# A-Andrews/Muzero-Hanoi

Measured on AMD Instinct MI355X. Metric: MCTS sims/sec (node) 4-disk Hanoi, 50 sims/move, 65k root batch; 1/2/4/8 GPU, higher is better.
Workload: dtype fp32

## Files before the change

muzero-hanoi_amd/csrc/mzh_wave.hip:

```cpp
#include "mzh_device.h"
#include "mzh_internal.h"
#include "mzh_mcts.h"

#define MZW_WAVES 4
#define MZW_DC 16

struct MzwNX {
  uint16_t N;
  int16_t X;
};
struct __align__(128) MzwBlock {
  MzwNX nx[6];
  float R[6];
  float P[6];
  double W[6];
  uint32_t pad[2];
};
static_assert(sizeof(MzwBlock) == 128, "block layout");

template <int ROOTS>
struct MzwWave {
  double rW[6][ROOTS];
  double rP[6][ROOTS];
  float rR[6][ROOTS];
  int rN[6][ROOTS];
  int rX[6][ROOTS];
  double pcW[MZW_DC][ROOTS];
  float pcR[MZW_DC][ROOTS];
  int pcN[MZW_DC][ROOTS];
  uint16_t path[MZW_DC][ROOTS];
};

static __host__ __device__ inline size_t mzw_hdr_bytes(int S) {
  size_t b = sizeof(float) * MZH_A * MZH_F + sizeof(double) * 2 * (size_t)(S + 3);
  return (b + 15) & ~(size_t)15;
}

__device__ __forceinline__ void mzw_wave_sync() {
  __builtin_amdgcn_fence(__ATOMIC_RELEASE, "wavefront");
  __builtin_amdgcn_wave_barrier();
  __builtin_amdgcn_fence(__ATOMIC_ACQUIRE, "wavefront");
}

__device__ __forceinline__ float mzw_max4g(float v) {
  float a, b;
  mzh_pair16(v, a, b);
  v = __builtin_fmaxf(a, b);
  mzh_pair32(v, a, b);
  return __builtin_fmaxf(a, b);
}
__device__ __forceinline__ float mzw_min4g(float v) {
  float a, b;
  mzh_pair16(v, a, b);
  v = __builtin_fminf(a, b);
  mzh_pair32(v, a, b);
  return __builtin_fminf(a, b);
}
__device__ __forceinline__ float mzw_add16(float v) {
  float a, b;
  mzh_pair16(v, a, b);
  return a + b;
}
__device__ __forceinline__ float mzw_add32(float v) {
  float a, b;
  mzh_pair32(v, a, b);
  return a + b;
}

__device__ __forceinline__ floatx4 mzw_ld4(__amdgpu_buffer_rsrc_t r, int voff, int soff) {
  return __builtin_bit_cast(floatx4, __builtin_amdgcn_raw_buffer_load_b128(r, voff, soff, 0));
}

template <int NT, int KB1, int NO, bool OH, bool B32 = false, int WS = 0>
__device__ __forceinline__ void mzw_chain(const MzhWMlp& L, __amdgpu_buffer_rsrc_t rw, const floatx4 (&x)[NT][4],
                                          const float* const (&oh)[NT], floatx4 (&out)[NO][NT], floatx4* b2, int lane,
                                          float* p32 = nullptr, floatx4* wst = nullptr, int next_soff = 0) {
  constexpr int FR = KB1 + NO;
  static_assert(WS == 0 || WS >= FR, "chained buffer too small");
  const int g = lane >> 4;
  const int vs = 16 * lane, vb = 16 * g;
#pragma unroll
  for (int ot = 0; ot < NO; ++ot)
#pragma unroll
    for (int n = 0; n < NT; ++n) out[ot][n] = floatx4{0.f, 0.f, 0.f, 0.f};
  floatx4 wloc[WS > 0 ? 1 : FR];
  floatx4* w = WS > 0 ? wst : wloc;
  if constexpr (WS == 0) {
#pragma unroll
    for (int f = 0; f < FR; ++f) w[f] = mzw_ld4(rw, vs, L.soff + f * 1024);
  }
#pragma unroll
  for (int ot = 0; ot < NO; ++ot) b2[ot] = mzw_ld4(rw, vb, L.b2off + 64 * ot);
  float a32[NT];
#pragma unroll
  for (int n = 0; n < NT; ++n) a32[n] = 0.0f;
#pragma unroll 2
  for (int ht = 0; ht < 16; ++ht) {
    const int sn = (WS > 0 && ht == 15) ? next_soff : L.soff + (ht + 1) * FR * 1024;
    const floatx4 b = mzw_ld4(rw, vb, L.b1off + 64 * ht);
    floatx4 w32 = {0.f, 0.f, 0.f, 0.f};
    if (B32) w32 = mzw_ld4(rw, vb, L.w32off + 64 * ht);
    floatx4 o[NT];
#pragma unroll
    for (int n = 0; n < NT; ++n)
      o[n] = OH ? *reinterpret_cast<const floatx4*>(oh[n] + 16 * ht) : floatx4{0.f, 0.f, 0.f, 0.f};
    floatx4 acc[NT];
#pragma unroll
    for (int n = 0; n < NT; ++n) acc[n] = floatx4{0.f, 0.f, 0.f, 0.f};
#pragma unroll
    for (int kb = 0; kb < KB1; ++kb) {
#pragma unroll
      for (int t = 0; t < 4; ++t)
#pragma unroll
        for (int n = 0; n < NT; ++n)
          acc[n] = __builtin_amdgcn_mfma_f32_16x16x4f32(w[kb][t], x[n][kb][t], acc[n], 0, 0, 0);
      w[kb] = mzw_ld4(rw, vs, sn + kb * 1024);
      __builtin_amdgcn_sched_barrier(0);
    }
    floatx4 hid[NT];
#pragma unroll
    for (int n = 0; n < NT; ++n) {
#pragma unroll
      for (int i = 0; i < 4; ++i) {
        float v = acc[n][i];
        if (OH) v = v + o[n][i];
        v = v + b[i];
        hid[n][i] = v > 0.0f ? v : 0.0f;
      }
    }
#pragma unroll
    for (int t = 0; t < 4; ++t) {
#pragma unroll
      for (int ot = 0; ot < NO; ++ot)
#pragma unroll
        for (int n = 0; n < NT; ++n)
          out[ot][n] = __builtin_amdgcn_mfma_f32_16x16x4f32(w[KB1 + ot][t], hid[n][t], out[ot][n], 0, 0, 0);
      if (B32) {
#pragma unroll
        for (int n = 0; n < NT; ++n) a32[n] = __builtin_fmaf(hid[n][t], w32[t], a32[n]);
        if (NT > 1) asm("" : "+v"(a32[0]));
      }
    }
#pragma unroll
    for (int ot = 0; ot < NO; ++ot) w[KB1 + ot] = mzw_ld4(rw, vs, sn + (KB1 + ot) * 1024);
    __builtin_amdgcn_sched_barrier(0);
  }
  if constexpr (WS > FR) {
#pragma unroll
    for (int f = FR; f < WS; ++f) w[f] = mzw_ld4(rw, vs, next_soff + f * 1024);
  }
  if (B32) {
#pragma unroll
    for (int n = 0; n < NT; ++n) p32[n] = a32[n];
  }
}

template <int NT, int NO>
__device__ __forceinline__ void mzw_bias2(floatx4 (&out)[NO][NT], const floatx4* b2) {
#pragma unroll
  for (int ot = 0; ot < NO; ++ot) {
    const floatx4 b = b2[ot];
#pragma unroll
    for (int n = 0; n < NT; ++n)
#pragma unroll
      for (int i = 0; i < 4; ++i) out[ot][n][i] = out[ot][n][i] + b[i];
  }
}

template <int NT>
__device__ __forceinline__ void mzw_normalize(const floatx4 (&hp)[4][NT], int n, floatx4 (&hn)[NT][4]) {
  float mn = hp[0][n][0], mx = hp[0][n][0];
#pragma unroll
  for (int ot = 0; ot < 4; ++ot)
#pragma unroll
    for (int i = 0; i < 4; ++i) {
      const float v = hp[ot][n][i];
      mn = __builtin_fminf(v, mn);
      mx = __builtin_fmaxf(v, mx);
    }
  mn = mzw_min4g(mn);
  mx = mzw_max4g(mx);
  const float d = (mx - mn) + 9.999999939225290290778502821922302246094e-09f;
  const float y = 1.0f / d;
  const float lim = __builtin_fmaxf(d < __builtin_inff() ? d * 0x1p-99f : 0.0f, 0x1p-100f);
  unsigned amin = 0xFFFFFFFFu;
#pragma unroll
  for (int ot = 0; ot < 4; ++ot)
#pragma unroll
    for (int i = 0; i < 4; ++i) {
      const float a = hp[ot][n][i] - mn;
      amin = min(amin, __float_as_uint(a) - 1u);
      const float q = a * y;
      hn[n][ot][i] = __builtin_fmaf(__builtin_fmaf(-q, d, a), y, q);
    }
  const bool slow = amin < __float_as_uint(lim) - 1u;
  if (__builtin_expect(__ballot(slow) != 0, 0)) {
#pragma unroll
    for (int ot = 0; ot < 4; ++ot)
#pragma unroll
      for (int i = 0; i < 4; ++i) hn[n][ot][i] = (hp[ot][n][i] - mn) / d;
  }
}

template <int NT, int NO>
__device__ __forceinline__ float mzw_head(const floatx4 (&l)[NO][NT], int n, int lane, float p32 = 0.0f,
                                          float b32 = 0.0f) {
  const int g = lane >> 4;
  if constexpr (NO == 1) {
    return __shfl(l[0][n][0], lane & 15);
  } else {
  static_assert(NO == 2, "33-bin heads: two tiles + the bin-32 chains");
  const bool v8 = g == 0;
  float L[9];
#pragma unroll
  for (int s = 0; s < 8; ++s) L[s] = l[s >> 2][n][s & 3];
  L[8] = mzw_add32(mzw_add16(p32)) + b32;
  float m = L[0];
#pragma unroll
  for (int s = 1; s < 8; ++s) m = __builtin_fmaxf(L[s], m);
  if (v8) m = __builtin_fmaxf(L[8], m);
  m = mzw_max4g(m);
  float e[9];
#pragma unroll
  for (int s = 0; s < 8; ++s) e[s] = mzh_expf_np(L[s] - m);
  e[8] = mzh_expf_np(L[8] - m);
  e[8] = v8 ? e[8] : 0.0f;
  float s0 = e[0];
  s0 = s0 + e[2];
  s0 = s0 + e[4];
  s0 = s0 + e[6];
  if (v8) s0 = s0 + e[8];
  float s1 = e[1];
  s1 = s1 + e[3];
  s1 = s1 + e[5];
  s1 = s1 + e[7];
  float t = s0 + s1;
  t = mzw_add16(t);
  t = mzw_add32(t);
  const float y = 1.0f / t;
  float lmin = L[0];
#pragma unroll
  for (int s = 1; s < 8; ++s) lmin = __builtin_fminf(L[s], lmin);
  if (v8) lmin = __builtin_fminf(L[8], lmin);
  const bool slow = lmin - m < -65.0f;
  float pk[9];
#pragma unroll
  for (int s = 0; s < 9; ++s) {
    const float q = e[s] * y;
    pk[s] = __builtin_fmaf(__builtin_fmaf(-q, t, e[s]), y, q);
  }
  if (__builtin_expect(__ballot(slow) != 0, 0)) {
#pragma unroll
    for (int s = 0; s < 9; ++s) pk[s] = e[s] / t;
  }
  float pr[9];
#pragma unroll
  for (int s = 0; s < 9; ++s) pr[s] = pk[s] * (float)(2 * g + (s & 1) + 8 * (s >> 1) - 16);
  float x0 = pr[0];
  x0 = x0 + pr[2];
  x0 = x0 + pr[4];
  x0 = x0 + pr[6];
  if (v8) x0 = x0 + pr[8];
  float x1 = pr[1];
  x1 = x1 + pr[3];
  x1 = x1 + pr[5];
  x1 = x1 + pr[7];
  float xs = x0 + x1;
  xs = mzw_add16(xs);
  xs = mzw_add32(xs);
  return mzh_signed_parabolic(xs);
  }
}

__device__ __forceinline__ floatx4 mzw_policy(const floatx4 l, int lane) {
  const int g = lane >> 4;
  const bool ok01 = g < 2, ok23 = g == 0;
  float m = -__builtin_inff();
  if (ok01) {
    m = __builtin_fmaxf(l[0], m);
    m = __builtin_fmaxf(l[1], m);
  }
  if (ok23) {
    m = __builtin_fmaxf(l[2], m);
    m = __builtin_fmaxf(l[3], m);
  }
  m = mzw_max4g(m);
  const float x0 = mzh_expf_np(l[0] - m), x1 = mzh_expf_np(l[1] - m);
  const float x2 = mzh_expf_np(l[2] - m), x3 = mzh_expf_np(l[3] - m);
  const float e0 = ok01 ? x0 : 0.0f, e1 = ok01 ? x1 : 0.0f;
  const float e2 = ok23 ? x2 : 0.0f, e3 = ok23 ? x3 : 0.0f;
  float t = (e0 + e1) + (e2 + e3);
  t = mzw_add16(t);
  const float y = 1.0f / t;
  float lmin = __builtin_inff();
  if (ok01) lmin = __builtin_fminf(__builtin_fminf(l[0], l[1]), lmin);
  if (ok23) lmin = __builtin_fminf(__builtin_fminf(l[2], l[3]), lmin);
  const bool slow = lmin - m < -65.0f;
  auto mdiv = [&](float a) {
    const float q = a * y;
    return __builtin_fmaf(__builtin_fmaf(-q, t, a), y, q);
  };
  floatx4 p;
  p[0] = mdiv(e0);
  p[1] = mdiv(e1);
  p[2] = mdiv(e2);
  p[3] = mdiv(e3);
  if (__builtin_expect(__ballot(slow) != 0, 0)) {
    p[0] = e0 / t;
    p[1] = e1 / t;
    p[2] = e2 / t;
    p[3] = e3 / t;
  }
  return p;
}

__device__ __forceinline__ int mzw_pick_pair(const float (&u)[3], int half, int tie, int& firstTie, int& extra) {
  float m = u[0];
  m = __builtin_fmaxf(u[1], m);
  m = __builtin_fmaxf(u[2], m);
  float a, b;
  mzh_pair32(m, a, b);
  const float M = __builtin_fmaxf(a, b);
  int mask = 0;
#pragma unroll
  for (int j = 0; j < 3; ++j) mask |= (u[j] == M ? 1 : 0) << j;
  mask <<= 3 * half;
  const auto r = __builtin_amdgcn_permlane32_swap((unsigned)mask, (unsigned)mask, false, false);
  return mzh_tie_pick(r[0] | r[1], tie, firstTie, extra);
}

template <int NC>
struct MzwCols {
  int root[NC];
  bool valid[NC];
  int en[NC], an[NC];
  int prow[NC];
  float val[NC], rew[NC];
  floatx4 cpi[NC];
};

template <int NT, bool REPLAY, bool SUP33>
__global__ __launch_bounds__(MZW_WAVES * 64, 2) void mzh_wave_kernel(MzhWNet net, MzhSearchParams p) {
  constexpr int NOV = SUP33 ? 2 : 1;
  constexpr int ROOTS = 16 * NT;
  const float* const noh[NT] = {};
  extern __shared__ __align__(16) unsigned char smem_raw[];
  const int S = p.S;
  float* ohl = reinterpret_cast<float*>(smem_raw);
  double* table = reinterpret_cast<double*>(smem_raw + sizeof(float) * MZH_A * MZH_F);
  MzwWave<ROOTS>* wsa = reinterpret_cast<MzwWave<ROOTS>*>(smem_raw + mzw_hdr_bytes(S));
  const int tid = threadIdx.x, lane = tid & 63;
  const int wave = __builtin_amdgcn_readfirstlane(tid >> 6);
  const int g = lane >> 4, col = lane & 15;
  const __amdgpu_buffer_rsrc_t rw = mzh_rsrc(net.wbase);

  if (!REPLAY)
    for (int i = tid; i < MZH_A * MZH_F; i += MZW_WAVES * 64) ohl[i] = net.oh[i];
  double* inv = table + (S + 3);
  for (int i = tid; i < S + 3; i += MZW_WAVES * 64) {
    table[i] = i < S + 2 ? p.table[i] : 0.0;
    inv[i] = 1.0 / (double)i;
  }
  __syncthreads();
  const int wr0 = (blockIdx.x * MZW_WAVES + wave) * ROOTS;
  if (wr0 >= p.B) return;
  MzwWave<ROOTS>& ws = wsa[wave];
  const double disc = p.discount;
  const bool noised = p.noise != nullptr;
  const size_t E = (size_t)p.E;

  const int rho = lane & 31;
  const int half = lane >> 5;
  const int rroot = wr0 + rho;
  const bool rvalid = rho < ROOTS && rroot < p.B;
  const int tb0 = (rvalid ? rroot : 0) * p.E;
  auto TB = [&](int e) -> MzwBlock& { return reinterpret_cast<MzwBlock*>(p.tree)[(size_t)(unsigned)(tb0 + e)]; };
  MzhMinMax mm;
  if (rvalid && p.minmax_in)
    mm.set(p.minmax_in[2 * rroot], p.minmax_in[2 * rroot + 1]);
  else
    mm.set(-__builtin_inf(), __builtin_inf());
  int firstTie = 0, extra = 0, steps = 0, rootN = 0, depth = 0;
  int leaf = 0;
  int lsum = 0;
  double rootW = 0.0;
  const int tie = (rvalid && p.tie_idx) ? p.tie_idx[rroot] : 0;
  const bool memo = !REPLAY && p.memo_h != nullptr;
  int sigma = -1;
  unsigned pid = 0;
  unsigned cnt = 0;
  const bool grow = memo && p.memo_link != nullptr;
  const bool glog = grow && p.memo_log != nullptr && p.memo_ctr[0] < p.memo_cap;
  if (memo && rvalid) {
    const unsigned* orow = reinterpret_cast<const unsigned*>(p.obs) + (size_t)rroot * p.in_dim;
    int sg = 0, w3 = 1;
    bool ok = true;
    for (int i = 0; 3 * i + 2 < p.in_dim; ++i, w3 *= 3) {
      const unsigned a0 = orow[3 * i], a1 = orow[3 * i + 1], a2 = orow[3 * i + 2];
      const unsigned one = 0x3F800000u;
      const int n1 = (a0 == one) + (a1 == one) + (a2 == one), n0 = (a0 == 0u) + (a1 == 0u) + (a2 == 0u);
      ok = ok && n1 == 1 && n0 == 2;
      sg += w3 * (a1 == one ? 1 : a2 == one ? 2 : 0);
    }
    sigma = ok ? sg : -1;
  }

  int croot[NT];
  bool cvalid[NT];
#pragma unroll
  for (int n = 0; n < NT; ++n) {
    croot[n] = wr0 + 16 * n + col;
    cvalid[n] = croot[n] < p.B;
  }

  floatx4 rpi[NT];
  const bool rtab = memo && __ballot(rvalid && sigma < 0) == 0;
  if (!REPLAY && rtab) {
#pragma unroll
    for (int n = 0; n < NT; ++n) {
      const int sg = __shfl(sigma, 16 * n + col);
      rpi[n] = floatx4{0.f, 0.f, 0.f, 0.f};
      if (cvalid[n] && g < 2) {
        const float* rec = p.memo_rec + (size_t)sg * p.memo_K * 8 + 4 * g;
        if (g == 0) {
          rpi[n] = *reinterpret_cast<const floatx4*>(rec);
        } else {
          rpi[n][0] = rec[0];
          rpi[n][1] = rec[1];
        }
      }
    }
  } else if (!REPLAY) {
    floatx4 hreg[NT][4];
    floatx4 x[NT][4];
#pragma unroll
    for (int n = 0; n < NT; ++n)
#pragma unroll
      for (int kb = 0; kb < 4; ++kb)
#pragma unroll
        for (int t = 0; t < 4; ++t) {
          const int k = 16 * kb + 4 * t + g;
          x[n][kb][t] = (cvalid[n] && k < p.in_dim) ? p.obs[(size_t)croot[n] * p.in_dim + k] : 0.0f;
        }
    floatx4 hp[4][NT];
    floatx4 b2[4];
    switch (net.rep.kb1) {
      case 1: mzw_chain<NT, 1, 4, false>(net.rep, rw, x, noh, hp, b2, lane); break;
      case 2: mzw_chain<NT, 2, 4, false>(net.rep, rw, x, noh, hp, b2, lane); break;
      case 3: mzw_chain<NT, 3, 4, false>(net.rep, rw, x, noh, hp, b2, lane); break;
      default: mzw_chain<NT, 4, 4, false>(net.rep, rw, x, noh, hp, b2, lane); break;
    }
    mzw_bias2<NT, 4>(hp, b2);
#pragma unroll
    for (int n = 0; n < NT; ++n) {
      mzw_normalize<NT>(hp, n, hreg);
      if (cvalid[n]) {
        floatx4* dst = reinterpret_cast<floatx4*>(p.htree + ((size_t)croot[n] * E) * MZH_H) + g;
#pragma unroll
        for (int kb = 0; kb < 4; ++kb) dst[4 * kb] = hreg[n][kb];
      }
    }
    floatx4 pl[1][NT];
    mzw_chain<NT, 4, 1, false>(net.pol, rw, hreg, noh, pl, b2, lane);
    mzw_bias2<NT, 1>(pl, b2);
    floatx4 vl[NOV][NT];
    mzw_chain<NT, 4, NOV, false>(net.val, rw, hreg, noh, vl, b2, lane);
    (void)vl;
#pragma unroll
    for (int n = 0; n < NT; ++n) rpi[n] = mzw_policy(pl[0][n], lane);
  }
  if (g < 2) {
#pragma unroll
    for (int n = 0; n < NT; ++n)
#pragma unroll
      for (int i = 0; i < 4; ++i) {
        const int c = 4 * g + i;
        if (c < MZH_A && cvalid[n]) {
          const float pr = REPLAY ? p.rp_root_pi[(size_t)croot[n] * MZH_A + c] : rpi[n][i];
          ws.rP[c][16 * n + col] =
              mzh_root_prior(pr, noised, p.eps, noised ? p.noise[(size_t)croot[n] * MZH_A + c] : 0.0);
        }
      }
  }
  if (lane < ROOTS) {
#pragma unroll
    for (int c = 0; c < MZH_A; ++c) {
      ws.rW[c][rho] = 0.0;
      ws.rR[c][rho] = 0.0f;
      ws.rN[c][rho] = 0;
      ws.rX[c][rho] = -1;
    }
  }
  mzw_wave_sync();

  MzwCols<NT> cf;
#pragma unroll
  for (int n = 0; n < NT; ++n) {
    cf.root[n] = cvalid[n] ? croot[n] : 0;
    cf.valid[n] = cvalid[n];
    cf.prow[n] = -1;
  }
  MzwCols<1> cp;

  floatx4 wst[8];
  if (!REPLAY) {
#pragma unroll
    for (int f = 0; f < 8; ++f) wst[f] = mzw_ld4(rw, 16 * lane, net.dyn.soff + f * 1024);
  }
  MZH_STAMP_DECL
  auto phase_select = [&](int s, auto ex) {
    (void)s;
    constexpr bool exact = decltype(ex)::value;
    if (rvalid) {
      const bool has = mm.has();
      const double mmin = mm.mmin, den = mm.den, dinv = mm.dinv;
      float u[3];
      const double tr = table[rootN];
#pragma unroll
      for (int j = 0; j < 3; ++j) {
        const int c = 3 * half + j;
        u[j] = mzh_ucb(ws.rN[c][rho], ws.rW[c][rho], ws.rR[c][rho], ws.rP[c][rho], noised || p.np1, tr, disc, has,
                       mmin, den, dinv, inv, exact);
      }
      int pick = mzw_pick_pair(u, half, tie, firstTie, extra);
      int Np = ws.rN[pick][rho], X = ws.rX[pick][rho];
      ws.path[0][rho] = (uint16_t)pick;
      ws.pcW[0][rho] = ws.rW[pick][rho];
      ws.pcR[0][rho] = ws.rR[pick][rho];
      ws.pcN[0][rho] = Np;
      int e = 0, d = 1;
      pid = 0;
      constexpr bool kPF = NT == 1;
      int pf0 = 0, pf1 = 0, pf2 = 0;
      while (X >= 0 && d <= S) {
        e = X;
        pid = 6u * pid + (unsigned)pick + 1u;
        int nx;
        double Wp;
        float Rp;
        {
          const unsigned char* blk = reinterpret_cast<const unsigned char*>(&TB(e));
          const uint3 hnx = *reinterpret_cast<const uint3*>(blk + 12 * half);
          const uint3 hR = *reinterpret_cast<const uint3*>(blk + 24 + 12 * half);
          const uint3 hP = *reinterpret_cast<const uint3*>(blk + 48 + 12 * half);
          typedef unsigned int u32x4_a8 __attribute__((ext_vector_type(4), aligned(8)));
          const u32x4_a8 hW01 = *reinterpret_cast<const u32x4_a8*>(blk + 72 + 24 * half);
          const uint2 hW2 = *reinterpret_cast<const uint2*>(blk + 88 + 24 * half);
          const int hn[3] = {(int)hnx.x, (int)hnx.y, (int)hnx.z};
          const float hr[3] = {__uint_as_float(hR.x), __uint_as_float(hR.y), __uint_as_float(hR.z)};
          const float hp[3] = {__uint_as_float(hP.x), __uint_as_float(hP.y), __uint_as_float(hP.z)};
          const double hw[3] = {__hiloint2double((int)hW01.y, (int)hW01.x), __hiloint2double((int)hW01.w, (int)hW01.z),
                                __hiloint2double((int)hW2.y, (int)hW2.x)};
          if (kPF) {
            asm volatile("" ::"v"(pf0), "v"(pf1), "v"(pf2));
            const int x0 = hn[0] >> 16, x1 = hn[1] >> 16, x2 = hn[2] >> 16;
            pf0 = *reinterpret_cast<const int*>(&TB(x0 >= 0 ? x0 : e));
            pf1 = *reinterpret_cast<const int*>(&TB(x1 >= 0 ? x1 : e));
            pf2 = *reinterpret_cast<const int*>(&TB(x2 >= 0 ? x2 : e));
          }
          const double tn = table[Np];
  #pragma unroll
          for (int j = 0; j < 3; ++j) u[j] = mzh_ucb(hn[j] & 0xFFFF, hw[j], hr[j], (double)hp[j], p.np1, tn, disc, has, mmin, den, dinv, inv, exact);
          pick = mzw_pick_pair(u, half, tie, firstTie, extra);
          const int jl = pick - 3 * half;
          int cn = hn[0];
          float cr = hr[0];
          double cw = hw[0];
  #pragma unroll
          for (int q = 1; q < 3; ++q)
            if (jl == q) {
              cn = hn[q];
              cr = hr[q];
              cw = hw[q];
            }
          auto take = [&](unsigned v) {
            const auto r = __builtin_amdgcn_permlane32_swap(v, v, false, false);
            return pick >= 3 ? r[1] : r[0];
          };
          nx = (int)take((unsigned)cn);
          Rp = __uint_as_float(take(__float_as_uint(cr)));
          const long long wb = __double_as_longlong(cw);
          Wp = __hiloint2double((int)take((unsigned)(wb >> 32)), (int)take((unsigned)(wb & 0xFFFFFFFFll)));
        }
        Np = nx & 0xFFFF;
        X = nx >> 16;
        const uint16_t slot = (uint16_t)(e * 8 + pick);
        if (d < MZW_DC) {
          ws.path[d][rho] = slot;
          ws.pcW[d][rho] = Wp;
          ws.pcR[d][rho] = Rp;
          ws.pcN[d][rho] = Np;
        } else {
          p.pathx[(size_t)rroot * E + d] = slot;
        }
        ++d;
      }
      if (kPF) asm volatile("" ::"v"(pf0), "v"(pf1), "v"(pf2));
      depth = d;
      leaf = (leaf & ~0x3FFFF) | (e * 8 + pick);
      steps += d;
    }
    if (p.lockstep_levels) {
      int m = rvalid ? depth - 1 : 0;
#pragma unroll
      for (int off = 32; off > 0; off >>= 1) m = max(m, __shfl_xor(m, off));
      lsum += m;
    }
  };

  auto phase_mlp = [&](int s, auto& C) {
    if (REPLAY) return;
    constexpr int NC = sizeof(C.root) / sizeof(int);
    const float* const nohc[NC] = {};
    floatx4 rl[NOV][NC], pl[1][NC], vl[NOV][NC];
    floatx4 x[NC][4];
#pragma unroll
    for (int n = 0; n < NC; ++n) {
      const float* row = C.prow[n] >= 0 ? p.memo_h + (size_t)C.prow[n] * MZH_H
                                        : p.htree + ((size_t)C.root[n] * E + C.en[n]) * MZH_H;
      const floatx4* src = reinterpret_cast<const floatx4*>(row) + g;
#pragma unroll
      for (int kb = 0; kb < 4; ++kb) x[n][kb] = src[4 * kb];
    }
    floatx4 hreg[NC][4];
    floatx4 hp[4][NC];
    const float* ohp[NC];
#pragma unroll
    for (int n = 0; n < NC; ++n) ohp[n] = ohl + C.an[n] * MZH_F + 4 * g;
    MZH_STAMP(10);
    floatx4 b2[4];
    mzw_chain<NC, 4, 4, true, false, 8>(net.dyn, rw, x, ohp, hp, b2, lane, nullptr, wst, net.rwd.soff);
    mzw_bias2<NC, 4>(hp, b2);
    MZH_STAMP(5);
    floatx4 hx[NC][4];
#pragma unroll
    for (int n = 0; n < NC; ++n)
#pragma unroll
      for (int kb = 0; kb < 4; ++kb) hx[n][kb] = hp[kb][n];
    float r32[NC], v32[NC];
    mzw_chain<NC, 4, NOV, false, SUP33, 8>(net.rwd, rw, hx, nohc, rl, b2, lane, r32, wst, net.pol.soff);
    mzw_bias2<NC, NOV>(rl, b2);
    MZH_STAMP(6);
#pragma unroll
    for (int n = 0; n < NC; ++n) C.rew[n] = mzw_head<NC, NOV>(rl, n, lane, SUP33 ? r32[n] : 0.0f, net.rwd.b32);
    MZH_STAMP(11);
#pragma unroll
    for (int n = 0; n < NC; ++n) {
      mzw_normalize<NC>(hp, n, hreg);
      if (C.valid[n]) {
        floatx4* dst = reinterpret_cast<floatx4*>(p.htree + ((size_t)C.root[n] * E + s + 1) * MZH_H) + g;
#pragma unroll
        for (int kb = 0; kb < 4; ++kb) dst[4 * kb] = hreg[n][kb];
      }
    }
    MZH_STAMP(7);
    mzw_chain<NC, 4, 1, false, false, 8>(net.pol, rw, hreg, nohc, pl, b2, lane, nullptr, wst, net.val.soff);
    mzw_bias2<NC, 1>(pl, b2);
#pragma unroll
    for (int n = 0; n < NC; ++n) C.cpi[n] = mzw_policy(pl[0][n], lane);
    MZH_STAMP(8);
    mzw_chain<NC, 4, NOV, false, SUP33, 8>(net.val, rw, hreg, nohc, vl, b2, lane, v32, wst, net.dyn.soff);
    mzw_bias2<NC, NOV>(vl, b2);
    MZH_STAMP(9);
#pragma unroll
    for (int n = 0; n < NC; ++n) C.val[n] = mzw_head<NC, NOV>(vl, n, lane, SUP33 ? v32[n] : 0.0f, net.val.b32);
  };

  auto phase_blocks = [&](int s, auto& C, bool own, int hrow) {
    constexpr int NC = sizeof(C.root) / sizeof(int);
    unsigned trow[NC];
#pragma unroll
    for (int n = 0; n < NC; ++n) trow[n] = own ? (unsigned)(__shfl(hrow, 16 * n + col) + 1) : 0u;
#pragma unroll
    for (int n = 0; n < NC; ++n) {
      if (!C.valid[n]) continue;
      uint4* nb = reinterpret_cast<uint4*>(reinterpret_cast<MzwBlock*>(p.tree) + (size_t)C.root[n] * E + s + 1);
      const uint32_t nx = 0xFFFF0000u;
      uint4 c0, c1;
      if (g == 0) {
        c0 = make_uint4(nx, nx, nx, nx);
        c1 = make_uint4(__float_as_uint(C.cpi[n][0]), __float_as_uint(C.cpi[n][1]), __float_as_uint(C.cpi[n][2]),
                        __float_as_uint(C.cpi[n][3]));
      } else if (g == 1) {
        c0 = make_uint4(nx, nx, 0u, 0u);
        c1 = make_uint4(__float_as_uint(C.cpi[n][0]), __float_as_uint(C.cpi[n][1]), 0u, 0u);
      } else {
        c0 = make_uint4(0u, 0u, 0u, 0u);
        c1 = make_uint4(0u, 0u, g == 3 ? trow[n] : 0u, 0u);
      }
      const int k0 = g < 3 ? g : 6, k1 = g < 3 ? g + 3 : 7;
      nb[k0] = c0;
      nb[k1] = c1;
    }
  };

  auto phase_head = [&](int s, bool fromrec, float vcol, float rcol, int hrow) {
    if (rvalid) {
      const int enew = s + 1;
      const int leafE = (leaf & 0x3FFFF) >> 3, leafA = leaf & 7;
      float vv, rr;
      if (REPLAY || fromrec) {
        const uint4* rec = reinterpret_cast<const uint4*>(
            REPLAY ? p.rp_sim + ((size_t)s * p.B + rroot) * 8 : p.memo_rec + (size_t)hrow * 8);
        const uint4 r0 = rec[0], r1 = rec[1];
        rr = __uint_as_float(r1.z);
        vv = __uint_as_float(r1.w);
        uint4* nb = reinterpret_cast<uint4*>(&TB(enew));
        const uint32_t nx = 0xFFFF0000u;
        const uint4 z = make_uint4(0u, 0u, 0u, 0u);
        const uint4 c7 = REPLAY ? z : make_uint4(0u, 0u, (unsigned)(hrow + 1), 0u);
        const bool h1 = half != 0;
        const uint32_t nx0 = h1 ? 0u : nx;
        nb += 4 * half;
        nb[0] = make_uint4(h1 ? r1.x : nx, h1 ? r1.y : nx, nx0, nx0);
        nb[1] = make_uint4(nx0, nx0, 0u, 0u);
        nb[2] = z;
        nb[3] = make_uint4(h1 ? 0u : r0.x, h1 ? 0u : r0.y, h1 ? c7.z : r0.z, h1 ? 0u : r0.w);
      } else {
        vv = vcol;
        rr = rcol;
        if (!REPLAY && glog && sigma >= 0 && hrow < 0 && (leaf >> 18) < p.memo_logcap) {
          int ro = rroot;
          asm volatile("" : "+v"(ro));
          if (!half)
            p.memo_log[(unsigned)(ro * p.memo_logcap + (leaf >> 18))] =
                make_uint4((unsigned)enew, (unsigned)(leaf & 0x3FFFF), __float_as_uint(vv), __float_as_uint(rr));
          leaf += 1 << 18;
        }
      }
      const bool st = !half;
      if (st) {
        if (leafE == 0) {
          ws.rX[leafA][rho] = enew;
          ws.rR[leafA][rho] = rr;
        } else {
          TB(leafE).nx[leafA].X = (int16_t)enew;
          TB(leafE).R[leafA] = rr;
        }
      }
      MZH_STAMP(12);
      double v = (double)vv;
      double lmax = -__builtin_inf(), lmin = __builtin_inf();
      auto load_lds = [&](int j, int& slot, double& W, float& R, int& N) {
        slot = ws.path[j][rho];
        W = ws.pcW[j][rho];
        R = ws.pcR[j][rho];
        N = ws.pcN[j][rho];
      };
      auto load_hbm = [&](int j, int& slot, double& W, float& R, int& N) {
        slot = p.pathx[(size_t)rroot * E + j];
        const int e = slot >> 3, a = slot & 7;
        W = TB(e).W[a];
        R = TB(e).R[a];
        N = TB(e).nx[a].N;
      };
      int slot;
      double Wj;
      float Rj;
      int Nj;
      auto node = [&](int j, double& Wn, int& Nn) {
        const double rw = (j == depth - 1) ? (double)rr : (double)Rj;
        Wn = Wj + v;
        Nn = Nj + 1;
        const double q = rw + disc * mzh_div(Wn, (double)Nn, inv[Nn]);
        lmax = q > lmax ? q : lmax;
        lmin = q < lmin ? q : lmin;
        v = rw + disc * v;
      };
      if (depth - 1 < MZW_DC) load_lds(depth - 1, slot, Wj, Rj, Nj);
      else load_hbm(depth - 1, slot, Wj, Rj, Nj);
      int j = depth - 1;
      auto hbm_node = [&](int jn) {
        const int e = slot >> 3, a = slot & 7;
        double Wn;
        int Nn;
        node(jn, Wn, Nn);
        if (st) {
          TB(e).W[a] = Wn;
          TB(e).nx[a].N = (uint16_t)Nn;
        }
      };
      for (; j >= 1; --j) {
        int slot_n, Nj_n;
        double Wj_n;
        float Rj_n;
        if (j - 1 < MZW_DC) load_lds(j - 1, slot_n, Wj_n, Rj_n, Nj_n);
        else load_hbm(j - 1, slot_n, Wj_n, Rj_n, Nj_n);
        hbm_node(j);
        slot = slot_n;
        Wj = Wj_n;
        Rj = Rj_n;
        Nj = Nj_n;
      }
      {
        const int a = slot & 7;
        double Wn;
        int Nn;
        node(0, Wn, Nn);
        if (st) {
          ws.rW[a][rho] = Wn;
          ws.rN[a][rho] = Nn;
        }
      }
      rootW = rootW + v;
      rootN = rootN + 1;
      const double q = 0.0 + disc * mzh_div(rootW, (double)rootN, inv[rootN]);
      lmax = q > lmax ? q : lmax;
      lmin = q < lmin ? q : lmin;
      mm.update(lmax, lmin);
    }
  };

  for (int s = 0; s < S; ++s) {
    MZH_STAMP(4);
    if (__builtin_expect(mzh_need_exact(rvalid && mm.has(), mm.den), 0))
      phase_select(s, MzhBool<true>{});
    else
      phase_select(s, MzhBool<false>{});
    MZH_STAMP(0);
    __builtin_amdgcn_s_setprio(1);
    int mode = 2, nm = 0;
    unsigned mask = 0;
    bool hit = false;
    int prow_r = -1, hrow = -1;
    const int leafE = (leaf & 0x3FFFF) >> 3, leafA = leaf & 7;
    if (memo && sigma >= 0) {
      if (depth - 1 <= p.memo_D) prow_r = sigma * p.memo_K + (int)pid;
      else if (grow) prow_r = (int)TB(leafE).pad[0] - 1;
      if (depth <= p.memo_D) {
        hrow = sigma * p.memo_K + (int)(6u * pid + (unsigned)leafA + 1u);
      } else if (grow && prow_r >= 0) {
        const int l = p.memo_link[prow_r * 6 + leafA];
        hrow = l > 0 ? l : -1;
      }
    }
    if (memo) {
      hit = hrow >= 0;
      mask = __builtin_amdgcn_readfirstlane((unsigned)__ballot(rvalid && !hit));
      nm = __popc(mask);
      mode = nm == 0 ? 0 : (NT == 2 && nm <= 16) ? 1 : 2;
      cnt = __builtin_amdgcn_readfirstlane(cnt + (mode == 0 ? 1u : mode == 1 ? 0x10000u : 0u));
    }
    MZH_STAMP(3);
    float vcol = 0.0f, rcol = 0.0f;
    if (mode == 2) {
      if (!REPLAY) {
#pragma unroll
        for (int n = 0; n < NT; ++n) {
          const int lf = __shfl(leaf, 16 * n + col);
          cf.en[n] = (lf & 0x3FFFF) >> 3;
          cf.an[n] = lf & 7;
          if (memo) cf.prow[n] = __shfl(prow_r, 16 * n + col);
        }
        phase_mlp(s, cf);
        vcol = cf.val[0];
        rcol = cf.rew[0];
#pragma unroll
        for (int n = 1; n < NT; ++n)
          if ((rho >> 4) == n) {
            vcol = cf.val[n];
            rcol = cf.rew[n];
          }
      }
    } else if constexpr (NT == 2) {
     if (mode == 1) {
      const int rank = __popc(mask & ((1u << rho) - 1u));
      const bool missl = (mask >> rho) & 1u;
      const int dest = half ? lane : (missl ? rank : nm + rho - rank);
      const int rsel = __builtin_amdgcn_ds_permute(dest << 2, rho);
      const bool pv = col < nm;
      const int rs = __shfl(rsel, col);
      const int r = pv ? rs : (int)__builtin_ctz(mask);
      cp.root[0] = wr0 + r;
      cp.valid[0] = pv;
      const int lf = __shfl(leaf, r);
      cp.en[0] = (lf & 0x3FFFF) >> 3;
      cp.an[0] = lf & 7;
      cp.prow[0] = __shfl(prow_r, r);
      phase_mlp(s, cp);
      vcol = __shfl(cp.val[0], rank);
      rcol = __shfl(cp.rew[0], rank);
     }
    }
    __builtin_amdgcn_s_setprio(0);
    MZH_STAMP(1);
    if (!REPLAY) {
      if (mode == 2) phase_blocks(s, cf, true, hrow);
      else if (NT == 2 && mode == 1) phase_blocks(s, cp, false, -1);
    }
    phase_head(s, mode != 2 && hit, vcol, rcol, hrow);
    MZH_STAMP(2);
    __builtin_amdgcn_fence(__ATOMIC_ACQ_REL, "workgroup");
    __builtin_amdgcn_wave_barrier();
  }

  if (p.lockstep_levels && lane == 0) p.lockstep_levels[blockIdx.x * MZW_WAVES + wave] = lsum;
  if (memo && lane == 0) {
    const unsigned nskip = cnt & 0xFFFFu, npack = cnt >> 16;
    atomicAdd(p.memo_cnt + 0, (unsigned long long)nskip);
    atomicAdd(p.memo_cnt + 1, (unsigned long long)npack);
    atomicAdd(p.memo_cnt + 2, (unsigned long long)((unsigned)S - nskip - npack));
    if (p.memo_logn && blockIdx.x == 0 && wave == 0) p.memo_ctr[1] = p.memo_ctr[0];
  }
  if (!rvalid || half) return;
  if (!REPLAY && p.memo_logn) p.memo_logn[rroot] = leaf >> 18;
  int vis[MZH_A];
  for (int a = 0; a < MZH_A; ++a) vis[a] = ws.rN[a][rho];
  mzh_write_results(p, rroot, vis, rootW, rootN, mm.mmax, mm.mmin, extra, steps, depth, [&](int j) {
    return j < MZW_DC ? (int)ws.path[j][rho] : (int)p.pathx[(size_t)rroot * E + j];
  });
}

size_t mzh_wave_smem_bytes(int S, int nt) {
  return mzw_hdr_bytes(S) + (nt == 1 ? sizeof(MzwWave<16>) : sizeof(MzwWave<32>)) * MZW_WAVES;
}

template <int NT, bool REPLAY, bool SUP33>
static hipError_t launch_wave_t(const MzhWNet& net, const MzhSearchParams& p, hipStream_t stream) {
  const size_t smem = mzh_wave_smem_bytes(p.S, NT);
  hipError_t e = hipFuncSetAttribute(reinterpret_cast<const void*>(&mzh_wave_kernel<NT, REPLAY, SUP33>),
                                     hipFuncAttributeMaxDynamicSharedMemorySize, (int)smem);
  if (e != hipSuccess) return e;
  const int per_wg = MZW_WAVES * 16 * NT;
  const int grid = (p.B + per_wg - 1) / per_wg;
  hipLaunchKernelGGL((mzh_wave_kernel<NT, REPLAY, SUP33>), dim3(grid), dim3(MZW_WAVES * 64), smem, stream, net, p);
  return hipGetLastError();
}

template <int NT>
static hipError_t launch_wave_nt(const MzhSearchPlan& pl, const MzhWNet& net, const MzhSearchParams& p, hipStream_t stream) {
  if (pl.replay) return pl.sup33 ? launch_wave_t<NT, true, true>(net, p, stream) : launch_wave_t<NT, true, false>(net, p, stream);
  return pl.sup33 ? launch_wave_t<NT, false, true>(net, p, stream) : launch_wave_t<NT, false, false>(net, p, stream);
}

hipError_t mzh_launch_wave_search(const MzhSearchPlan& pl, const MzhWNet& net, const MzhSearchParams& p, hipStream_t stream) {
  return pl.nt == 1 ? launch_wave_nt<1>(pl, net, p, stream) : launch_wave_nt<2>(pl, net, p, stream);
}

__global__ __launch_bounds__(256) void mzh_memo_level_kernel(const float4* hprev, float4* xin, int32_t* act, long long n) {
  const long long i = (long long)blockIdx.x * 256 + threadIdx.x;
  if (i >= n * 16) return;
  const long long r = i >> 4;
  xin[i] = hprev[(r / 6) * 16 + (i & 15)];
  if ((i & 15) == 0) act[r] = (int32_t)(r % 6);
}
__global__ __launch_bounds__(256) void mzh_memo_scatter_kernel(const float* h, const float* pi, const float* reward,
                                                               const float* value, long long n, long long per_state,
                                                               long long K, long long first_id, float* memo_h,
                                                               float* memo_rec) {
  const long long i = (long long)blockIdx.x * 256 + threadIdx.x;
  if (i >= n * 64) return;
  const long long r = i >> 6;
  const int pos = (int)(i & 63);
  const long long row = (r / per_state) * K + first_id + (r % per_state);
  const int kb = pos >> 4, gg = (pos >> 2) & 3, t = pos & 3;
  memo_h[row * 64 + pos] = h[r * 64 + 16 * kb + 4 * t + gg];
  if (pos < 8) memo_rec[row * 8 + pos] = pos < 6 ? pi[r * 6 + pos] : pos == 6 ? reward[r] : value[r];
}
hipError_t mzh_launch_memo_level(const float* hprev, float* xin, int32_t* act, long long n, hipStream_t stream) {
  const long long blocks = (n * 16 + 255) / 256;
  hipLaunchKernelGGL(mzh_memo_level_kernel, dim3((unsigned)blocks), dim3(256), 0, stream,
                     reinterpret_cast<const float4*>(hprev), reinterpret_cast<float4*>(xin), act, n);
  return hipGetLastError();
}
hipError_t mzh_launch_memo_scatter(const float* h, const float* pi, const float* reward, const float* value, long long n,
                                   long long per_state, long long K, long long first_id, float* memo_h, float* memo_rec,
                                   hipStream_t stream) {
  const long long blocks = (n * 64 + 255) / 256;
  hipLaunchKernelGGL(mzh_memo_scatter_kernel, dim3((unsigned)blocks), dim3(256), 0, stream, h, pi, reward, value, n,
                     per_state, K, first_id, memo_h, memo_rec);
  return hipGetLastError();
}

__global__ __launch_bounds__(256) void mzh_memo_harvest_kernel(MzhHarvestParams h) {
  const int root = blockIdx.x * 256 + threadIdx.x;
  if (root >= h.B) return;
  int n = h.logn[root];
  if (n <= 0) return;
  n = min(n, h.logcap);
  MzwBlock* tb = reinterpret_cast<MzwBlock*>(h.tree) + (size_t)root * h.E;
  const uint4* log = h.log + (size_t)root * h.logcap;
  for (int i = 0; i < n; ++i) {
    const uint4 en = log[i];
    const int e = (int)en.x, pe = (int)(en.y >> 3), a = (int)(en.y & 7u);
    if (e < 1 || e >= h.E || pe < 1 || pe >= h.E || a >= MZH_A) continue;
    const int prow = (int)tb[pe].pad[0] - 1;
    if (prow < 0 || prow >= h.base + h.cap) continue;
    int32_t* lk = h.link + prow * 6 + a;
    const int old = atomicCAS(lk, MZH_LINK_NONE, MZH_LINK_CLAIM);
    if (old > 0) {
      tb[e].pad[0] = (uint32_t)(old + 1);
      continue;
    }
    if (old != MZH_LINK_NONE) continue;
    const int r = atomicAdd(h.ctr, 1);
    if (r >= h.cap) {
      atomicSub(h.ctr, 1);
      atomicExch(lk, MZH_LINK_NONE);
      return;
    }
    const int row = h.base + r;
    const float4* src = reinterpret_cast<const float4*>(h.htree + ((size_t)root * h.E + e) * MZH_H);
    float4* dst = reinterpret_cast<float4*>(h.memo_h + (size_t)row * MZH_H);
#pragma unroll
    for (int k = 0; k < MZH_H / 4; ++k) dst[k] = src[k];
    const float* P = tb[e].P;
    float4* rec = reinterpret_cast<float4*>(h.memo_rec + (size_t)row * 8);
    rec[0] = make_float4(P[0], P[1], P[2], P[3]);
    rec[1] = make_float4(P[4], P[5], __uint_as_float(en.w), __uint_as_float(en.z));
    atomicExch(lk, row);
    tb[e].pad[0] = (uint32_t)(row + 1);
  }
}
hipError_t mzh_launch_memo_harvest(const MzhHarvestParams& h, hipStream_t stream) {
  hipLaunchKernelGGL(mzh_memo_harvest_kernel, dim3((unsigned)((h.B + 255) / 256)), dim3(256), 0, stream, h);
  return hipGetLastError();
}

#ifdef MZH_STAMPS
extern "C" int mzh_diag_wave_stamps(unsigned long long* host) {
  if (hipMemcpyFromSymbol(host, HIP_SYMBOL(mzh_stamp_acc), sizeof(mzh_stamp_acc)) != hipSuccess) return -2;
  static unsigned long long zero[8][MZH_NSTAMP] = {};
  if (hipMemcpyToSymbol(HIP_SYMBOL(mzh_stamp_acc), zero, sizeof(zero)) != hipSuccess) return -2;
  return 0;
}
#endif
```

Before: 2.741 billion.

## Reorganize tree node block into per-half AoS units with fused backup writes

Changes the 128-byte tree block from SoA arrays (N/X, R, P, W) into two 64-byte halves of three 16-byte child units plus a P triple and a memo row index. Each lane half now fetches its children with four aligned 16-byte loads instead of several unaligned pieces. Backup writes one packed 16-byte unit with W, N, X and R together, which replaces the separate leaf X/R write and the scattered field stores. The memo row is read from the half just loaded, so the extra block access is gone. This touches selection, expansion, backup and harvest all at once, so any mismatch in offsets or in the duplicated row1 value could corrupt the tree.

```diff
diff --git a/muzero-hanoi_amd/csrc/mzh_wave.hip b/muzero-hanoi_amd/csrc/mzh_wave.hip
--- a/muzero-hanoi_amd/csrc/mzh_wave.hip
+++ b/muzero-hanoi_amd/csrc/mzh_wave.hip
@@ -5,17 +5,22 @@
 #define MZW_WAVES 4
 #define MZW_DC 16
 
-struct MzwNX {
+struct MzwUnit {
+  double W;
   uint16_t N;
   int16_t X;
+  float R;
+};
+struct MzwHalf {
+  MzwUnit c[3];
+  float P[3];
+  uint32_t row1;
 };
 struct __align__(128) MzwBlock {
-  MzwNX nx[6];
-  float R[6];
-  float P[6];
-  double W[6];
-  uint32_t pad[2];
+  MzwHalf h[2];
 };
+static_assert(sizeof(MzwUnit) == 16 && sizeof(MzwHalf) == 64, "block layout");
+static_assert(__builtin_offsetof(MzwHalf, P) == 48 && __builtin_offsetof(MzwHalf, row1) == 60, "block layout");
 static_assert(sizeof(MzwBlock) == 128, "block layout");
 
 template <int ROOTS>
@@ -388,6 +393,7 @@
   const bool memo = !REPLAY && p.memo_h != nullptr;
   int sigma = -1;
   unsigned pid = 0;
+  unsigned row1 = 0;
   unsigned cnt = 0;
   const bool grow = memo && p.memo_link != nullptr;
   const bool glog = grow && p.memo_log != nullptr && p.memo_ctr[0] < p.memo_cap;
@@ -530,6 +536,7 @@
       ws.pcN[0][rho] = Np;
       int e = 0, d = 1;
       pid = 0;
+      row1 = 0;
       constexpr bool kPF = NT == 1;
       int pf0 = 0, pf1 = 0, pf2 = 0;
       while (X >= 0 && d <= S) {
@@ -539,18 +546,16 @@
         double Wp;
         float Rp;
         {
-          const unsigned char* blk = reinterpret_cast<const unsigned char*>(&TB(e));
-          const uint3 hnx = *reinterpret_cast<const uint3*>(blk + 12 * half);
-          const uint3 hR = *reinterpret_cast<const uint3*>(blk + 24 + 12 * half);
-          const uint3 hP = *reinterpret_cast<const uint3*>(blk + 48 + 12 * half);
-          typedef unsigned int u32x4_a8 __attribute__((ext_vector_type(4), aligned(8)));
-          const u32x4_a8 hW01 = *reinterpret_cast<const u32x4_a8*>(blk + 72 + 24 * half);
-          const uint2 hW2 = *reinterpret_cast<const uint2*>(blk + 88 + 24 * half);
-          const int hn[3] = {(int)hnx.x, (int)hnx.y, (int)hnx.z};
-          const float hr[3] = {__uint_as_float(hR.x), __uint_as_float(hR.y), __uint_as_float(hR.z)};
+          const uint4* hb = reinterpret_cast<const uint4*>(&TB(e).h[half]);
+          uint4 u0 = hb[0], u1 = hb[1], u2 = hb[2], hP = hb[3];
+          asm("" : "+v"(u0.x), "+v"(u0.y), "+v"(u0.z), "+v"(u0.w));
+          asm("" : "+v"(u1.x), "+v"(u1.y), "+v"(u2.x), "+v"(u2.y));
+          row1 = hP.w;
+          const int hn[3] = {(int)u0.z, (int)u1.z, (int)u2.z};
+          const float hr[3] = {__uint_as_float(u0.w), __uint_as_float(u1.w), __uint_as_float(u2.w)};
           const float hp[3] = {__uint_as_float(hP.x), __uint_as_float(hP.y), __uint_as_float(hP.z)};
-          const double hw[3] = {__hiloint2double((int)hW01.y, (int)hW01.x), __hiloint2double((int)hW01.w, (int)hW01.z),
-                                __hiloint2double((int)hW2.y, (int)hW2.x)};
+          const double hw[3] = {__hiloint2double((int)u0.y, (int)u0.x), __hiloint2double((int)u1.y, (int)u1.x),
+                                __hiloint2double((int)u2.y, (int)u2.x)};
           if (kPF) {
             asm volatile("" ::"v"(pf0), "v"(pf1), "v"(pf2));
             const int x0 = hn[0] >> 16, x1 = hn[1] >> 16, x2 = hn[2] >> 16;
@@ -671,25 +676,25 @@
     unsigned trow[NC];
 #pragma unroll
     for (int n = 0; n < NC; ++n) trow[n] = own ? (unsigned)(__shfl(hrow, 16 * n + col) + 1) : 0u;
+    float p3[NC];
+#pragma unroll
+    for (int n = 0; n < NC; ++n) {
+      float hi;
+      mzh_pair16(C.cpi[n][3], p3[n], hi);
+      (void)hi;
+    }
 #pragma unroll
     for (int n = 0; n < NC; ++n) {
       if (!C.valid[n]) continue;
       uint4* nb = reinterpret_cast<uint4*>(reinterpret_cast<MzwBlock*>(p.tree) + (size_t)C.root[n] * E + s + 1);
-      const uint32_t nx = 0xFFFF0000u;
-      uint4 c0, c1;
-      if (g == 0) {
-        c0 = make_uint4(nx, nx, nx, nx);
-        c1 = make_uint4(__float_as_uint(C.cpi[n][0]), __float_as_uint(C.cpi[n][1]), __float_as_uint(C.cpi[n][2]),
-                        __float_as_uint(C.cpi[n][3]));
-      } else if (g == 1) {
-        c0 = make_uint4(nx, nx, 0u, 0u);
-        c1 = make_uint4(__float_as_uint(C.cpi[n][0]), __float_as_uint(C.cpi[n][1]), 0u, 0u);
-      } else {
-        c0 = make_uint4(0u, 0u, 0u, 0u);
-        c1 = make_uint4(0u, 0u, g == 3 ? trow[n] : 0u, 0u);
-      }
-      const int k0 = g < 3 ? g : 6, k1 = g < 3 ? g + 3 : 7;
-      nb[k0] = c0;
+      const uint4 eu = make_uint4(0u, 0u, 0xFFFF0000u, 0u);
+      uint4 c1 = eu;
+      if (g == 0)
+        c1 = make_uint4(__float_as_uint(C.cpi[n][0]), __float_as_uint(C.cpi[n][1]), __float_as_uint(C.cpi[n][2]), trow[n]);
+      else if (g == 1)
+        c1 = make_uint4(__float_as_uint(p3[n]), __float_as_uint(C.cpi[n][0]), __float_as_uint(C.cpi[n][1]), trow[n]);
+      const int k0 = 4 * (g & 1) + (g >> 1), k1 = g < 2 ? 4 * g + 3 : k0 + 1;
+      nb[k0] = eu;
       nb[k1] = c1;
     }
   };
@@ -705,17 +710,13 @@
         const uint4 r0 = rec[0], r1 = rec[1];
         rr = __uint_as_float(r1.z);
         vv = __uint_as_float(r1.w);
-        uint4* nb = reinterpret_cast<uint4*>(&TB(enew));
-        const uint32_t nx = 0xFFFF0000u;
-        const uint4 z = make_uint4(0u, 0u, 0u, 0u);
-        const uint4 c7 = REPLAY ? z : make_uint4(0u, 0u, (unsigned)(hrow + 1), 0u);
+        uint4* nb = reinterpret_cast<uint4*>(&TB(enew).h[half]);
+        const uint4 eu = make_uint4(0u, 0u, 0xFFFF0000u, 0u);
         const bool h1 = half != 0;
-        const uint32_t nx0 = h1 ? 0u : nx;
-        nb += 4 * half;
-        nb[0] = make_uint4(h1 ? r1.x : nx, h1 ? r1.y : nx, nx0, nx0);
-        nb[1] = make_uint4(nx0, nx0, 0u, 0u);
-        nb[2] = z;
-        nb[3] = make_uint4(h1 ? 0u : r0.x, h1 ? 0u : r0.y, h1 ? c7.z : r0.z, h1 ? 0u : r0.w);
+        nb[0] = eu;
+        nb[1] = eu;
+        nb[2] = eu;
+        nb[3] = make_uint4(h1 ? r0.w : r0.x, h1 ? r1.x : r0.y, h1 ? r1.y : r0.z, REPLAY ? 0u : (unsigned)(hrow + 1));
       } else {
         vv = vcol;
         rr = rcol;
@@ -729,14 +730,9 @@
         }
       }
       const bool st = !half;
-      if (st) {
-        if (leafE == 0) {
-          ws.rX[leafA][rho] = enew;
-          ws.rR[leafA][rho] = rr;
-        } else {
-          TB(leafE).nx[leafA].X = (int16_t)enew;
-          TB(leafE).R[leafA] = rr;
-        }
+      if (st && leafE == 0) {
+        ws.rX[leafA][rho] = enew;
+        ws.rR[leafA][rho] = rr;
       }
       MZH_STAMP(12);
       double v = (double)vv;
@@ -750,9 +746,11 @@
       auto load_hbm = [&](int j, int& slot, double& W, float& R, int& N) {
         slot = p.pathx[(size_t)rroot * E + j];
         const int e = slot >> 3, a = slot & 7;
-        W = TB(e).W[a];
-        R = TB(e).R[a];
-        N = TB(e).nx[a].N;
+        uint4 un = reinterpret_cast<const uint4*>(&TB(e))[a + (a >= 3)];
+        asm("" : "+v"(un.x), "+v"(un.y), "+v"(un.z), "+v"(un.w));
+        W = __hiloint2double((int)un.y, (int)un.x);
+        R = __uint_as_float(un.w);
+        N = (int)(un.z & 0xFFFFu);
       };
       int slot;
       double Wj;
@@ -770,15 +768,20 @@
       if (depth - 1 < MZW_DC) load_lds(depth - 1, slot, Wj, Rj, Nj);
       else load_hbm(depth - 1, slot, Wj, Rj, Nj);
       int j = depth - 1;
+      int xn = enew;
       auto hbm_node = [&](int jn) {
         const int e = slot >> 3, a = slot & 7;
         double Wn;
         int Nn;
         node(jn, Wn, Nn);
         if (st) {
-          TB(e).W[a] = Wn;
-          TB(e).nx[a].N = (uint16_t)Nn;
+          const float rs = (jn == depth - 1) ? rr : Rj;
+          const long long wb = __double_as_longlong(Wn);
+          reinterpret_cast<uint4*>(&TB(e))[a + (a >= 3)] =
+              make_uint4((unsigned)(wb & 0xFFFFFFFFll), (unsigned)(wb >> 32), ((unsigned)Nn & 0xFFFFu) | ((unsigned)xn << 16),
+                         __float_as_uint(rs));
         }
+        xn = e;
       };
       for (; j >= 1; --j) {
         int slot_n, Nj_n;
@@ -823,10 +826,10 @@
     unsigned mask = 0;
     bool hit = false;
     int prow_r = -1, hrow = -1;
-    const int leafE = (leaf & 0x3FFFF) >> 3, leafA = leaf & 7;
+    const int leafA = leaf & 7;
     if (memo && sigma >= 0) {
       if (depth - 1 <= p.memo_D) prow_r = sigma * p.memo_K + (int)pid;
-      else if (grow) prow_r = (int)TB(leafE).pad[0] - 1;
+      else if (grow) prow_r = (int)row1 - 1;
       if (depth <= p.memo_D) {
         hrow = sigma * p.memo_K + (int)(6u * pid + (unsigned)leafA + 1u);
       } else if (grow && prow_r >= 0) {
@@ -984,12 +987,12 @@
     const uint4 en = log[i];
     const int e = (int)en.x, pe = (int)(en.y >> 3), a = (int)(en.y & 7u);
     if (e < 1 || e >= h.E || pe < 1 || pe >= h.E || a >= MZH_A) continue;
-    const int prow = (int)tb[pe].pad[0] - 1;
+    const int prow = (int)tb[pe].h[0].row1 - 1;
     if (prow < 0 || prow >= h.base + h.cap) continue;
     int32_t* lk = h.link + prow * 6 + a;
     const int old = atomicCAS(lk, MZH_LINK_NONE, MZH_LINK_CLAIM);
     if (old > 0) {
-      tb[e].pad[0] = (uint32_t)(old + 1);
+      tb[e].h[0].row1 = tb[e].h[1].row1 = (uint32_t)(old + 1);
       continue;
     }
     if (old != MZH_LINK_NONE) continue;
@@ -1004,12 +1007,12 @@
     float4* dst = reinterpret_cast<float4*>(h.memo_h + (size_t)row * MZH_H);
 #pragma unroll
     for (int k = 0; k < MZH_H / 4; ++k) dst[k] = src[k];
-    const float* P = tb[e].P;
+    const float *P = tb[e].h[0].P, *Q = tb[e].h[1].P;
     float4* rec = reinterpret_cast<float4*>(h.memo_rec + (size_t)row * 8);
-    rec[0] = make_float4(P[0], P[1], P[2], P[3]);
-    rec[1] = make_float4(P[4], P[5], __uint_as_float(en.w), __uint_as_float(en.z));
+    rec[0] = make_float4(P[0], P[1], P[2], Q[0]);
+    rec[1] = make_float4(Q[1], Q[2], __uint_as_float(en.w), __uint_as_float(en.z));
     atomicExch(lk, row);
-    tb[e].pad[0] = (uint32_t)(row + 1);
+    tb[e].h[0].row1 = tb[e].h[1].row1 = (uint32_t)(row + 1);
   }
 }
 hipError_t mzh_launch_memo_harvest(const MzhHarvestParams& h, hipStream_t stream) {
```

New measurement: 3.099 billion (median of 6 runs). 13.0% higher.
